# PlanNoa/video_super_resolution

Measured on AMD Instinct MI355X. Metric: HR frames/sec, 1080p->4K x4 VSR (LR 540x960 -> 2160x3840), VSR.forward end-to-end, higher is better.
Workload: dtype f16

## Files before the change

__graft_entry__.py:

```python
import os

os.environ.setdefault("MIOPEN_FIND_MODE", "2")
os.environ.setdefault("MIOPEN_DEBUG_ENABLE_AI_IMMED_MODE_FALLBACK", "0")
os.environ.setdefault("MIOPEN_LOG_LEVEL", "2")
import subprocess
import sys

ROOT = os.path.dirname(os.path.abspath(__file__))
if ROOT not in sys.path:
    sys.path.insert(0, ROOT)


def build() -> None:
    from video_super_resolution_amd import _lib
    _lib.build(verbose=True)
    subprocess.check_call(["make", "-s", "-C", os.path.join(ROOT, "oracle"), "_build/liboracle_native.so"])
    import video_super_resolution_amd
    missing = [s for s in _lib.declared_symbols() if not hasattr(_lib.load(), s)]
    if missing:
        raise RuntimeError(f"libvsr_hip.so lacks {missing}")
    xmissing = [s for s in _lib.declared_symbols() + _lib.declared_symbols(xcheck=True) if not hasattr(_lib.load_xcheck(), s)]
    if xmissing:
        raise RuntimeError(f"libvsr_hip_xcheck.so lacks {xmissing}")
    s3missing = [s for s in _lib.declared_symbols(s3=True) if not hasattr(_lib.load_s3(), s)]
    if s3missing:
        raise RuntimeError(f"libvsr_hip_s3.so lacks {s3missing}")
    s3tmissing = [s for s in _lib.declared_symbols(s3t=True) if not hasattr(_lib.load_s3t(), s)]
    if s3tmissing:
        raise RuntimeError(f"libvsr_hip_s3t.so lacks {s3tmissing}")


def smoke() -> None:
    import numpy as np
    import torch
    from oracle import native, vsr_oracle
    from video_super_resolution_amd import SRProjectionModule, ops
    from video_super_resolution_amd.weights import fill_module_

    assert torch.cuda.is_available(), "smoke() needs cuda:0"
    torch.cuda.set_device(0)
    rs = np.random.RandomState(0)
    img = rs.randn(1, 3, 32, 48).astype(np.float32)
    flow = (rs.randn(1, 2, 32, 48) * 4).astype(np.float32)
    got = ops.resample2d(torch.from_numpy(img).cuda(), torch.from_numpy(flow).cuda()).cpu().numpy()
    assert np.array_equal(got, native.resample2d(img, flow)), "flow warp differs from the oracle"

    sr = fill_module_(SRProjectionModule().eval(), seed=0, prefix="model.")
    x = torch.from_numpy(rs.randint(0, 256, (8, 3, 10, 12)).astype(np.float32))
    with torch.no_grad():
        ref = vsr_oracle.sr_forward({k: v for k, v in sr.state_dict().items()}, x).numpy()
    sr = sr.cuda()
    errs = {}
    for precision, bar in (("fp32", 1e-3), ("fp16", 5e-3)):
        sr.precision = precision
        out = sr(x.cuda()).cpu().numpy()
        errs[precision] = np.abs(out - ref).max() / np.abs(ref).max()
        assert errs[precision] < bar, f"SR forward ({precision}) differs from the oracle: {errs[precision]}"
    print(f"smoke ok: warp bit-exact, SR forward rel err fp32 {errs['fp32']:.2e}, fp16/MFMA {errs['fp16']:.2e}")


if __name__ == "__main__":
    build()
    if len(sys.argv) > 1 and sys.argv[1] == "smoke":
        smoke()
```

video_super_resolution_amd/_lib.py:

```python
from __future__ import annotations

import ctypes
import os
import re
import subprocess

import torch

_PKG = os.path.dirname(os.path.abspath(__file__))
_ROOT = os.path.dirname(_PKG)
LIB_PATH = os.path.join(_PKG, "libvsr_hip.so")
XLIB_PATH = os.path.join(_PKG, "libvsr_hip_xcheck.so")
HEADER_PATH = os.path.join(_ROOT, "include", "vsr_hip.h")
XHEADER_PATH = os.path.join(_ROOT, "include", "vsr_hip_xcheck.h")
GLIB_PATH = os.path.join(_PKG, "libvsr_hip_grad.so")
GHEADER_PATH = os.path.join(_ROOT, "include", "vsr_hip_grad.h")
S3LIB_PATH = os.path.join(_PKG, "libvsr_hip_s3.so")
S3HEADER_PATH = os.path.join(_ROOT, "include", "vsr_hip_s3.h")
S3TLIB_PATH = os.path.join(_PKG, "libvsr_hip_s3t.so")
S3THEADER_PATH = os.path.join(_ROOT, "include", "vsr_hip_s3t.h")
_lib = None
_xlib = None
_glib = None
_s3lib = None
_s3tlib = None
_use_x = os.environ.get("VSR_USE_XCHECK", "0") == "1" or bool(os.environ.get("VSR_TUNING", "").strip())


class VsrHipError(RuntimeError):
    pass


def build(verbose: bool = False) -> str:
    cmd = ["make", "-j4", "-C", os.path.join(_PKG, "csrc")]
    if not verbose:
        cmd.insert(1, "-s")
    subprocess.check_call(cmd)
    return LIB_PATH


def declared_symbols(xcheck: bool = False, grad: bool = False, s3: bool = False, s3t: bool = False) -> list:
    with open(S3THEADER_PATH if s3t else S3HEADER_PATH if s3 else GHEADER_PATH if grad else XHEADER_PATH if xcheck else HEADER_PATH) as f:
        text = re.sub(r"/\*.*?\*/", "", f.read(), flags=re.S)
    return sorted(set(re.findall(r"\b(vsr_[a-z0-9_]+)\s*\(", text)))


def _dlopen(path: str) -> ctypes.CDLL:
    if not os.path.exists(path):
        raise VsrHipError(
            f"{path} is missing: build it with `python -c 'import __graft_entry__ as g; g.build()'` "
            "(there is no CPU fallback for the device path)")
    return ctypes.CDLL(path)


def _open(path: str) -> ctypes.CDLL:
    lib = _dlopen(path)
    lib.vsr_last_error.restype = ctypes.c_char_p
    lib.vsr_last_route.restype = ctypes.c_char_p
    for fn in ("vsr_sr_query", "vsr_train_corr_dw_ws_floats", "vsr_train_prelu_bwd_ws_floats"):
        getattr(lib, fn).restype = ctypes.c_size_t
    if lib.vsr_abi_version() != 3:
        raise VsrHipError(f"{os.path.basename(path)}: ABI version mismatch")
    return lib


def load_xcheck() -> ctypes.CDLL:
    global _xlib
    if _xlib is None:
        lib = _open(XLIB_PATH)
        for t in os.environ.get("VSR_TUNING", "").split(","):
            if t.strip():
                lib.vsr_conv2d_tuning(int(t))
        _xlib = lib
    return _xlib


def load_grad() -> ctypes.CDLL:
    global _glib
    if _glib is None:
        lib = _dlopen(GLIB_PATH)
        lib.vsr_grad_last_error.restype = ctypes.c_char_p
        lib.vsr_last_error = lib.vsr_grad_last_error
        if lib.vsr_grad_abi_version() != 1:
            raise VsrHipError(f"{os.path.basename(GLIB_PATH)}: ABI version mismatch")
        _glib = lib
    return _glib


def load_s3() -> ctypes.CDLL:
    global _s3lib
    if _s3lib is None:
        lib = _dlopen(S3LIB_PATH)
        lib.vsr_s3_last_error.restype = ctypes.c_char_p
        lib.vsr_last_error = lib.vsr_s3_last_error
        lib.vsr_s3_query.restype = ctypes.c_size_t
        if lib.vsr_s3_abi_version() != 1:
            raise VsrHipError(f"{os.path.basename(S3LIB_PATH)}: ABI version mismatch")
        _s3lib = lib
    return _s3lib


def load_s3t() -> ctypes.CDLL:
    global _s3tlib
    if _s3tlib is None:
        lib = _dlopen(S3TLIB_PATH)
        lib.vsr_s3t_last_error.restype = ctypes.c_char_p
        lib.vsr_last_error = lib.vsr_s3t_last_error
        lib.vsr_s3t_query.restype = ctypes.c_size_t
        if lib.vsr_s3t_abi_version() != 1:
            raise VsrHipError(f"{os.path.basename(S3TLIB_PATH)}: ABI version mismatch")
        _s3tlib = lib
    return _s3tlib


def load() -> ctypes.CDLL:
    global _lib
    if _use_x:
        return load_xcheck()
    if _lib is None:
        _lib = _open(LIB_PATH)
    return _lib


class xcheck:

    def __enter__(self):
        global _use_x
        self._old, _use_x = _use_x, True
        return load_xcheck()

    def __exit__(self, *exc):
        global _use_x
        _use_x = self._old
        return False


Q_UTD_BLOB_BYTES, Q_UTD_STRIP_WIDTH, Q_UTD_S2_BLOB_BYTES, Q_UTD_S2_STRIP_WIDTH, Q_TAIL_S2_BLOB_BYTES = range(5)
Q_S3_BLOB_BYTES, Q_S3_STRIP_WIDTH = range(2)
Q_S3T_BLOB_BYTES, Q_S3T_BLOB_FOLD_BYTES, Q_S3T_STRIP_WIDTH = range(3)


def check(rc: int, what: str = "", lib=None) -> None:
    if rc != 0:
        libs = [lib] if lib is not None else [l for l in (load(), _lib, _xlib) if l is not None]
        msgs = []
        for l in libs:
            m = l.vsr_last_error().decode("utf-8", "replace")
            if m and m not in msgs:
                msgs.append(m)
        raise VsrHipError(f"{what or 'vsr'} failed ({rc}): {' | '.join(msgs)}")


def dptr(t: torch.Tensor, dtype=torch.float32) -> ctypes.c_void_p:
    if not t.is_cuda:
        raise VsrHipError("device path called with a CPU tensor (no CPU fallback exists)")
    if t.dtype != dtype:
        raise VsrHipError(f"expected {dtype}, got {t.dtype}")
    if not t.is_contiguous():
        raise VsrHipError("tensor must be contiguous")
    return ctypes.c_void_p(t.data_ptr())


def optr(t, dtype=torch.float32):
    return ctypes.c_void_p(0) if t is None else dptr(t, dtype)


_raw_stream = getattr(torch._C, "_cuda_getCurrentRawStream", None)


def raw_stream(index=None) -> int:
    if _raw_stream is not None:
        return _raw_stream(torch._C._cuda_getDevice() if index is None else index)
    return torch.cuda.current_stream(index).cuda_stream


def stream() -> ctypes.c_void_p:
    return ctypes.c_void_p(raw_stream())


def _first_cuda_tensor(objs):
    for o in objs:
        if isinstance(o, torch.Tensor):
            if o.is_cuda:
                return o
        elif isinstance(o, (list, tuple)):
            t = _first_cuda_tensor(o)
            if t is not None:
                return t
    return None


def on_device(fn):
    import functools

    @functools.wraps(fn)
    def wrapped(*args, **kwargs):
        t = _first_cuda_tensor(args)
        if t is None:
            t = _first_cuda_tensor(tuple(kwargs.values()))
        if t is None or t.device.index == torch.cuda.current_device():
            return fn(*args, **kwargs)
        with torch.cuda.device(t.device):
            return fn(*args, **kwargs)
    return wrapped


def cf(v: float) -> ctypes.c_float:
    return ctypes.c_float(float(v))


class _ChainStage(ctypes.Structure):
    _fields_ = [("inp", ctypes.c_void_p * 2), ("w", ctypes.c_void_p * 2), ("ldw", ctypes.c_int * 2), ("w_prev", ctypes.c_void_p),
                ("ldw_prev", ctypes.c_int), ("bias", ctypes.c_void_p), ("cmap", ctypes.c_void_p), ("slope", ctypes.c_float),
                ("out", ctypes.c_void_p)]


class Chain1x1(ctypes.Structure):
    _fields_ = [("nstages", ctypes.c_int), ("stage", _ChainStage * 3)]


_ROUTE_BATCH = os.environ.get("VSR_ROUTE_BATCH", "1") != "0"


class route_batch:

    def __init__(self, num: int, den: int):
        self.num, self.den = int(num), int(den)
        self.on = self.den > 0 and self.num > 0 and self.num != self.den and _ROUTE_BATCH

    def __enter__(self):
        if self.on:
            check(load().vsr_conv2d_route_batch(self.num, self.den), "conv2d_route_batch")
        return self

    def __exit__(self, *exc):
        if self.on:
            load().vsr_conv2d_route_batch(0, 0)
        return False


class serial_streams:
    on = False

    def __init__(self, enable: bool = True):
        self.enable = bool(enable)

    def __enter__(self):
        self._old, serial_streams.on = serial_streams.on, serial_streams.on or self.enable
        return self

    def __exit__(self, *exc):
        serial_streams.on = self._old
        return False


class EventTimer:

    def __init__(self):
        self.enabled = False
        self.only = None
        self._pairs = {}

    def reset(self):
        self._pairs = {}

    def start(self, name: str):
        if not self.enabled or (self.only is not None and name not in self.only):
            return None
        a = torch.cuda.Event(enable_timing=True)
        b = torch.cuda.Event(enable_timing=True)
        a.record()
        self._pairs.setdefault(name, []).append((a, b))
        return b

    @staticmethod
    def stop(tok):
        if tok is not None:
            tok.record()

    def summary(self):
        return {k: (len(v), sum(a.elapsed_time(b) for a, b in v) / len(v)) for k, v in self._pairs.items()}


TIMER = EventTimer()


class RouteLog:

    def __init__(self):
        self.enabled = False
        self.calls = []

    def note(self, label: str):
        if self.enabled:
            self.calls.append((label, load().vsr_last_route().decode()))

    def note_as(self, label: str, route: str):
        if self.enabled:
            self.calls.append((label, route))

    def last(self) -> str:
        return load().vsr_last_route().decode()

    def histogram(self):
        h = {}
        for _, r in self.calls:
            h[r] = h.get(r, 0) + 1
        return h


ROUTES = RouteLog()
```

video_super_resolution_amd/trunk_exec.py:

```python
from __future__ import annotations

import ctypes
import os

import torch
import torch.nn as nn
import torch.nn.functional as F

from . import _lib as L
from . import ops
from .depth import HOURGLASS
from .igemm import (ACT_LEAKY, ACT_NONE, ACT_RELU, HConv, HConvPairS2, HConvStem, HDeconv4s2, HFlowHead, HHourglassFront, SegMap, cached_zeros,
                    pad32, pool2x2, resize_add, to_nhwc_half)


def _fold(conv: nn.Conv2d, bn):
    w = conv.weight.detach().float()
    b = conv.bias.detach().float() if conv.bias is not None else torch.zeros(w.shape[0], device=w.device)
    if bn is not None:
        scale = torch.rsqrt(bn.running_var.float() + bn.eps)
        if bn.affine:
            scale = scale * bn.weight.detach().float()
        shift = -bn.running_mean.float() * scale
        if bn.affine:
            shift = shift + bn.bias.detach().float()
        w = w * scale.view(-1, 1, 1, 1)
        b = b * scale + shift
    return w, b


def _nchw(x):
    return x.permute(0, 3, 1, 2)


def _nhwc(x):
    return x.permute(0, 2, 3, 1).contiguous()


class _Inception:

    def __init__(self, mod):
        b0 = mod[0]
        w0, bb0 = _fold(b0[0], b0[1])
        ws, bs, self.kconvs = [], [], []
        mids, outs = [], []
        for j in (1, 2, 3):
            br = mod[j]
            w1, b1 = _fold(br[0], br[1])
            ws.append(w1)
            bs.append(b1)
            mids.append(w1.shape[0])
            wk, bk = _fold(br[3], br[4])
            outs.append(wk.shape[0])
            self.kconvs.append((wk, bk, br[3].kernel_size[0]))
        self.M = sum(mids)
        self.o0 = w0.shape[0]
        self.ctot = self.o0 + sum(outs)
        self.width = pad32(self.M + self.ctot)
        self.first = HConv(torch.cat(ws + [w0], 0), torch.cat(bs + [bb0], 0), act=ACT_RELU)
        packed = []
        moff, ooff = 0, self.M + self.o0
        for (wk, bk, k), mid, o in zip(self.kconvs, mids, outs):
            packed.append((HConv(wk, bk, pad=(k - 1) // 2, act=ACT_RELU), moff, ooff))
            moff += mid
            ooff += o
        self.kconvs = packed
        self.cin = w0.shape[1]

    dense_thin = os.environ.get("VSR_DENSE_THIN", "1") != "0"

    def branches(self, buf):
        if self.dense_thin and all(conv.cout == 16 for conv, _, _ in self.kconvs) and self.o0 == 16:
            N, H, W, _ = buf.shape
            outs = torch.empty((len(self.kconvs), N, H, W, 16), dtype=torch.float16, device=buf.device)
            for j, (conv, moff, _) in enumerate(self.kconvs):
                conv(buf, out=outs[j], out_coff=0, in_coff=moff)
            return SegMap([(buf, self.M)] + [(outs[j], 0) for j in range(len(self.kconvs))]), 0, self.ctot
        for conv, moff, ooff in self.kconvs:
            conv(buf, out=buf, out_coff=ooff, in_coff=moff)
        return buf, self.M, self.ctot

    def __call__(self, x, in_coff):
        N, H, W, _ = x.shape
        buf = torch.empty((N, H, W, self.width), dtype=torch.float16, device=x.device)
        if self.width != self.M + self.ctot:
            buf[..., self.M + self.ctot:] = 0
        self.first(x, out=buf, out_coff=0, in_coff=in_coff)
        return self.branches(buf)


class HourglassExec:
    fused_front = os.environ.get("VSR_HG_FRONT", "1") != "0"

    def __init__(self, netg: nn.Sequential):
        self.prog = self._build(HOURGLASS, netg)
        self.front = self._match_front(self.prog)

    @staticmethod
    def _match_front(prog):
        try:
            items = prog[1]
            stem, lvl = items[0], items[1]
            fan = lvl[1][0]
            arm_a, arm_b = fan[1]
            ok = (stem[0] == "stem" and stem[2] == 128 and lvl[0] == "S" and lvl[1][1] == "+" and len(lvl[1]) == 2 and fan[0] == "M" and
                  arm_a[0] == "S" and arm_a[1][0] == "max" and arm_b[0] == "S" and len(arm_b[1]) == 1 and arm_b[1][0][0] == "I" and
                  arm_b[1][0][1].cin == 128)
            return HHourglassFront(stem[1], arm_b[1][0][1].first) if ok else None
        except (IndexError, TypeError, ValueError, AttributeError):
            return None

    def _build(self, node, mod):
        if isinstance(node, str):
            return node
        tag = node[0]
        if tag == "S":
            items, children = [], list(mod)
            i = 0
            while i < len(node[1]):
                ch = node[1][i]
                if isinstance(ch, tuple) and ch[0] == "conv":
                    bn = children[i + 1] if i + 1 < len(children) and isinstance(children[i + 1], nn.BatchNorm2d) else None
                    j = i + (2 if bn is not None else 1)
                    relu = j < len(children) and isinstance(children[j], nn.ReLU)
                    w, b = _fold(children[i], bn)
                    if w.shape[1] <= 4 and w.shape[3] <= 8:
                        items.append(("stem", HConvStem(w, b, pad=ch[4], act=ACT_RELU if relu else ACT_NONE), ch[2]))
                    else:
                        items.append(("conv", HConv(w, b, pad=ch[4], act=ACT_RELU if relu else ACT_NONE), ch[2]))
                    i = j + (1 if relu else 0)
                    continue
                items.append(self._build(ch, children[i]))
                i += 1
            return ("S", items)
        if tag == "M":
            return ("M", [self._build(c, m) for c, m in zip(node[1], mod)])
        if tag == "I":
            return ("I", _Inception(mod))
        raise ValueError(node)

    def _side(self, dev, level):
        if L.serial_streams.on:
            return torch.cuda.current_stream(dev)
        key = (dev.type, dev.index)
        if getattr(self, "_side_key", None) != key:
            self._side_streams, self._side_key = {}, key
        if level not in self._side_streams:
            self._side_streams[level] = torch.cuda.Stream(device=dev)
        return self._side_streams[level]

    def _fan_out(self, subs, x, coff, c, level):
        if len(subs) != 2 or not self.concurrent:
            return [self._run(sub, x, coff, c, level + 1) for sub in subs]
        cur = torch.cuda.current_stream(x.device)
        side = self._side(x.device, level)
        side.wait_stream(cur)
        with torch.cuda.stream(side):
            first = self._run(subs[0], x, coff, c, level + 1)
            first[0].record_stream(cur)
        x.record_stream(side)
        second = self._run(subs[1], x, coff, c, level + 1)
        cur.wait_stream(side)
        return [first, second]

    concurrent = os.environ.get("VSR_HOURGLASS_STREAMS", "0") == "1"
    defer_up = True

    def _run(self, node, x, coff, c, level=0):
        if node == "max" or node == "avg":
            return pool2x2(x, coff, c, 0 if node == "max" else 1), 0, c
        if node == "up":
            return resize_add(x, coff, c, (2 * x.shape[1], 2 * x.shape[2])), 0, c
        tag = node[0]
        if tag == "conv":
            if node[2] == 1:
                N, H, W, _ = x.shape
                Ho, Wo = node[1].out_hw(H, W)
                out = node[1](x, in_coff=coff, out=torch.empty((N, Ho, Wo, 1), dtype=torch.float16, device=x.device))
            else:
                out = node[1](x, in_coff=coff)
            return out, 0, node[2]
        if tag == "stem":
            return node[1](x), 0, node[2]
        if tag == "I":
            buf, m, ctot = node[1](x, coff)
            return buf, m, ctot
        if tag == "S":
            items = node[1]
            for i, ch in enumerate(items):
                if ch == "+":
                    a, ca, na = x[0][:3]
                    b, cb, nb = x[1][:3]
                    a_up, b_up = len(x[0]) > 3, len(x[1]) > 3
                    out_hw = (b.shape[1] << b_up, b.shape[2] << b_up)
                    x, coff, c = resize_add(a, ca, nb, out_hw, b, cb, up2=a_up, b_up2=b_up), 0, nb
                elif isinstance(ch, tuple) and ch[0] == "M":
                    x = self._fan_out(ch[1], x, coff, c, level)
                elif ch == "up" and i == len(items) - 1 and self.defer_up:
                    return x, coff, c, "up2"
                else:
                    x, coff, c = self._run(ch, x, coff, c, level)
            return x, coff, c
        raise ValueError(node)

    @L.on_device
    @torch.no_grad()
    def __call__(self, frames_nhwc3: torch.Tensor) -> torch.Tensor:
        k, h, w, _ = frames_nhwc3.shape
        stem_first = self.prog[0] == "S" and isinstance(self.prog[1][0], tuple) and self.prog[1][0][0] == "stem"
        x = cached_zeros(self, "in", (k, h, w, 4 if stem_first else 32), frames_nhwc3.device)
        x[..., :3] = frames_nhwc3
        if self.front is not None and self.fused_front and h >= 2 and w >= 2:
            out, coff, c = self._run_fused_front(x)
        else:
            out, coff, c = self._run(self.prog, x, 0, 32)
        return out[..., coff:coff + 1].permute(0, 3, 1, 2).float()

    def _run_fused_front(self, x4):
        k, h, w, _ = x4.shape
        items = self.prog[1]
        arm_a, arm_b = items[1][1][0][1]
        inc = arm_b[1][0][1]
        buf = torch.empty((k, h, w, inc.width), dtype=torch.float16, device=x4.device)
        if inc.width != inc.M + inc.ctot:
            buf[..., inc.M + inc.ctot:] = 0
        pooled = torch.empty((k, h // 2, w // 2, 128), dtype=torch.float16, device=x4.device)
        self.front(x4, buf, pooled)
        a = self._run(("S", arm_a[1][1:]), pooled, 0, 128, 1)
        x, coff, c = self._run(("S", ["+"]), [a, inc.branches(buf)], 0, 0)
        return self._run(("S", items[2:]), x, coff, c)


def _cv(seq, stride=1, act=ACT_LEAKY, cin_pad=None):
    conv = seq[0] if isinstance(seq, nn.Sequential) else seq
    k = conv.kernel_size[0]
    return HConv(conv.weight, conv.bias, stride=conv.stride[0], pad=(k - 1) // 2, act=act, slope=0.1, cin_pad=cin_pad)


class _Refine:
    fused_heads = os.environ.get("VSR_FLOW_HEADS", "1") != "0"

    def __init__(self, net, with_inter: bool):
        self.with_inter = with_inter
        self.pred6 = _cv(net.predict_flow6, act=ACT_NONE)
        self.levels = []
        prev_pred = net.predict_flow6
        for lvl, cin_cat in ((5, 1026), (4, 770), (3, 386), (2, 194)):
            dec = getattr(net, f"deconv{lvl}")[0]
            up = getattr(net, f"upsampled_flow{lvl + 1}_to_{lvl}")
            item = dict(deconv=HDeconv4s2(dec.weight, dec.bias, act=ACT_LEAKY),
                        upflow=HDeconv4s2(up.weight, up.bias, act=ACT_NONE),
                        cat=pad32(cin_cat), dec_c=dec.weight.shape[1])
            pred = getattr(net, f"predict_flow{lvl}")
            if with_inter:
                item["inter"] = _cv(getattr(net, f"inter_conv{lvl}"), act=ACT_NONE, cin_pad=pad32(cin_cat))
                item["pred"] = _cv(pred, act=ACT_NONE)
            else:
                item["pred"] = _cv(pred, act=ACT_NONE, cin_pad=pad32(cin_cat))
            item["head_in"] = HFlowHead(prev_pred.weight, prev_pred.bias, up.weight, up.bias,
                                        cin_pad=None if (with_inter or lvl == 5) else self.levels[-1]["cat"])
            prev_pred = pred
            self.levels.append(item)
        self.head_last = HFlowHead(prev_pred.weight, prev_pred.bias, cin_pad=None if with_inter else self.levels[-1]["cat"])

    def alloc_cat(self, idx, N, H, W, dev):
        return cached_zeros(self, f"cat{idx}", (N, H, W, self.levels[idx]["cat"]), dev)

    def __call__(self, c6, cats, enc_c):
        if not self.fused_heads:
            flow = self.pred6(c6)
            src = c6
            for i, lv in enumerate(self.levels):
                cat = cats[i]
                lv["deconv"](src, out=cat, out_coff=enc_c[i])
                lv["upflow"](flow, out=cat, out_coff=enc_c[i] + lv["dec_c"])
                flow = lv["pred"](lv["inter"](cat)) if self.with_inter else lv["pred"](cat)
                src = cat
            return flow
        src = head_src = c6
        for i, lv in enumerate(self.levels):
            cat = cats[i]
            lv["deconv"](src, out=cat, out_coff=enc_c[i])
            lv["head_in"](head_src, up_out=cat, up_coff=enc_c[i] + lv["dec_c"])
            src = cat
            head_src = lv["inter"](cat) if self.with_inter else cat
        return self.head_last(head_src)


class _FlowNetSExec:
    def __init__(self, net, cin):
        c1 = net.conv1[0] if isinstance(net.conv1, nn.Sequential) else net.conv1
        self.conv1 = HConvPairS2(c1.weight, c1.bias, pad=(c1.kernel_size[0] - 1) // 2, act=ACT_LEAKY, slope=0.1) \
            if cin <= 16 and c1.stride[0] == 2 else _cv(net.conv1, cin_pad=pad32(cin))
        self.pair_input = isinstance(self.conv1, HConvPairS2)
        self.names = ["conv2", "conv3", "conv3_1", "conv4", "conv4_1", "conv5", "conv5_1", "conv6", "conv6_1"]
        self.convs = {n: _cv(getattr(net, n)) for n in self.names}
        self.refine = _Refine(net, with_inter=False)

    def __call__(self, x):
        N, H, W, _ = x.shape
        dev = x.device
        c1 = self.conv1(x)
        h2, w2 = H // 4, W // 4
        cats = [self.refine.alloc_cat(i, N, H >> (5 - i), W >> (5 - i), dev) for i in range(4)]
        self.convs["conv2"](c1, out=cats[3], out_coff=0)
        self.convs["conv3_1"](self.convs["conv3"](cats[3]), out=cats[2], out_coff=0)
        self.convs["conv4_1"](self.convs["conv4"](cats[2]), out=cats[1], out_coff=0)
        self.convs["conv5_1"](self.convs["conv5"](cats[1]), out=cats[0], out_coff=0)
        c6 = self.convs["conv6_1"](self.convs["conv6"](cats[0]))
        return self.refine(c6, cats, [512, 512, 256, 128])


class _FlowNetCExec:
    def __init__(self, net):
        c1 = net.conv1[0] if isinstance(net.conv1, nn.Sequential) else net.conv1
        self.conv1 = HConvStem(c1.weight, c1.bias, stride=c1.stride[0], pad=(c1.kernel_size[0] - 1) // 2, act=ACT_LEAKY, slope=0.1)
        self.conv2, self.conv3 = _cv(net.conv2), _cv(net.conv3)
        self.redir = _cv(net.conv_redir)
        self.conv3_1 = _cv(net.conv3_1, cin_pad=pad32(473))
        self.names = ["conv4", "conv4_1", "conv5", "conv5_1", "conv6", "conv6_1"]
        self.convs = {n: _cv(getattr(net, n)) for n in self.names}
        self.refine = _Refine(net, with_inter=False)

    def __call__(self, x6, both=None):
        B, H, W, _ = x6.shape
        dev = x6.device
        if both is None:
            both = cached_zeros(self, "both", (2 * B, H, W, 4), dev)
            both[:B, ..., :3] = x6[..., 0:3]
            both[B:, ..., :3] = x6[..., 3:6]
        c2 = self.conv2(self.conv1(both))
        c3 = self.conv3(c2)
        a3, b3 = c3[:B], c3[B:]
        h8, w8 = H // 8, W // 8
        cat31 = cached_zeros(self, "cat31", (B, h8, w8, pad32(473)), dev)
        self.redir(a3, out=cat31, out_coff=0)
        L.check(L.load().vsr_flownetc_corr_nhwc_f16(L.dptr(a3, torch.float16), L.dptr(b3, torch.float16), L.dptr(cat31, torch.float16),
                                                    cat31.shape[3], 32, B, h8, w8, c3.shape[3], L.stream()), "flownetc_corr")
        cats = [self.refine.alloc_cat(i, B, H >> (5 - i), W >> (5 - i), dev) for i in range(4)]
        cats[3][..., :128] = c2[:B]
        self.conv3_1(cat31, out=cats[2], out_coff=0)
        self.convs["conv4_1"](self.convs["conv4"](cats[2]), out=cats[1], out_coff=0)
        self.convs["conv5_1"](self.convs["conv5"](cats[1]), out=cats[0], out_coff=0)
        c6 = self.convs["conv6_1"](self.convs["conv6"](cats[0]))
        return self.refine(c6, cats, [512, 512, 256, 128])


class _FlowNetSDExec:
    def __init__(self, net):
        self.conv0 = _cv(net.conv0, cin_pad=32)
        self.names = ["conv1", "conv1_1", "conv2", "conv2_1", "conv3", "conv3_1", "conv4", "conv4_1", "conv5", "conv5_1",
                      "conv6", "conv6_1"]
        self.convs = {n: _cv(getattr(net, n)) for n in self.names}
        self.refine = _Refine(net, with_inter=True)

    def __call__(self, x6):
        N, H, W, _ = x6.shape
        dev = x6.device
        c = self.convs
        c0 = self.conv0(x6)
        c1 = c["conv1_1"](c["conv1"](c0))
        cats = [self.refine.alloc_cat(i, N, H >> (5 - i), W >> (5 - i), dev) for i in range(4)]
        c["conv2_1"](c["conv2"](c1), out=cats[3], out_coff=0)
        c["conv3_1"](c["conv3"](cats[3]), out=cats[2], out_coff=0)
        c["conv4_1"](c["conv4"](cats[2]), out=cats[1], out_coff=0)
        c["conv5_1"](c["conv5"](cats[1]), out=cats[0], out_coff=0)
        c6 = c["conv6_1"](c["conv6"](cats[0]))
        return self.refine(c6, cats, [512, 512, 256, 128])


class _FusionExec:
    def __init__(self, net):
        self.conv0 = _cv(net.conv0, cin_pad=32)
        self.conv1, self.conv1_1 = _cv(net.conv1), _cv(net.conv1_1)
        self.conv2, self.conv2_1 = _cv(net.conv2), _cv(net.conv2_1)
        self.pred2 = _cv(net.predict_flow2, act=ACT_NONE)
        self.deconv1 = HDeconv4s2(net.deconv1[0].weight, net.deconv1[0].bias, act=ACT_LEAKY)
        self.up21 = HDeconv4s2(net.upsampled_flow2_to_1.weight, net.upsampled_flow2_to_1.bias)
        self.inter1 = _cv(net.inter_conv1, act=ACT_NONE, cin_pad=pad32(162))
        self.pred1 = _cv(net.predict_flow1, act=ACT_NONE)
        self.deconv0 = HDeconv4s2(net.deconv0[0].weight, net.deconv0[0].bias, act=ACT_LEAKY, cin_pad=pad32(162))
        self.up10 = HDeconv4s2(net.upsampled_flow1_to_0.weight, net.upsampled_flow1_to_0.bias)
        self.inter0 = _cv(net.inter_conv0, act=ACT_NONE, cin_pad=pad32(82))
        self.pred0 = _cv(net.predict_flow0, act=ACT_NONE)
        self.head2 = HFlowHead(net.predict_flow2.weight, net.predict_flow2.bias, net.upsampled_flow2_to_1.weight, net.upsampled_flow2_to_1.bias)

    def __call__(self, x11):
        N, H, W, _ = x11.shape
        dev = x11.device
        cat0 = cached_zeros(self, "cat0", (N, H, W, pad32(82)), dev)
        cat1 = cached_zeros(self, "cat1", (N, H // 2, W // 2, pad32(162)), dev)
        self.conv0(x11, out=cat0, out_coff=0)
        self.conv1_1(self.conv1(cat0), out=cat1, out_coff=0)
        c2 = self.conv2_1(self.conv2(cat1))
        if _Refine.fused_heads:
            self.head2(c2, up_out=cat1, up_coff=160)
            self.deconv1(c2, out=cat1, out_coff=128)
        else:
            flow2 = self.pred2(c2)
            self.deconv1(c2, out=cat1, out_coff=128)
            self.up21(flow2, out=cat1, out_coff=160)
        flow1 = self.pred1(self.inter1(cat1))
        self.deconv0(cat1, out=cat0, out_coff=64)
        self.up10(flow1, out=cat0, out_coff=80)
        return self.pred0(self.inter0(cat0))


class FlowNet2Exec:
    def __init__(self, net):
        self.div_flow = net.div_flow
        self.c = _FlowNetCExec(net.flownetc)
        self.s1 = _FlowNetSExec(net.flownets_1, 12)
        self.s2 = _FlowNetSExec(net.flownets_2, 12)
        self.sd = _FlowNetSDExec(net.flownets_d)
        self.fusion = _FusionExec(net.flownetfusion)

    def _sd_stream(self, dev):
        if L.serial_streams.on:
            return torch.cuda.current_stream(dev)
        key = (dev.type, dev.index)
        if getattr(self, "_sd_key", None) != key:
            self._sd_side, self._sd_key = torch.cuda.Stream(device=dev), key
        return self._sd_side

    @staticmethod
    def _flow_nchw(t):
        return t[..., :2].permute(0, 3, 1, 2).float()

    @L.on_device
    @torch.no_grad()
    def __call__(self, inputs):
        B, _, _, H, W = inputs.shape
        frames = inputs.float().permute(0, 2, 3, 4, 1).reshape(2 * B, H, W, 3).contiguous()
        out = []
        for b0 in range(0, B, 4):
            nb = min(4, B - b0)
            out.append(self.run_pairs(frames[2 * b0:2 * (b0 + nb)], [(2 * i, 2 * i + 1) for i in range(nb)]))
        return self._flow_nchw(out[0] if len(out) == 1 else torch.cat(out, 0))

    @L.on_device
    @torch.no_grad()
    def run_pairs(self, frames, pairs, crop=None):
        lib = L.load()
        B = len(pairs)
        F_, h, w, _ = frames.shape
        y0, x0, H, W = crop or (0, 0, h, w)
        dev = frames.device
        frames = frames.contiguous()
        x = torch.empty((B, 6, H, W), dtype=torch.float32, device=dev)
        x6 = torch.empty((B, H, W, 32), dtype=torch.float16, device=dev)
        both = torch.empty((2 * B, H, W, 4), dtype=torch.float16, device=dev)
        ws = torch.empty(B * 128 * 3, dtype=torch.float32, device=dev)
        ia = (ctypes.c_int * B)(*[p[0] for p in pairs])
        ib = (ctypes.c_int * B)(*[p[1] for p in pairs])
        L.check(lib.vsr_flownet_prepare_pairs(L.dptr(frames), F_, h, w, ia, ib, B, y0, x0, H, W, L.dptr(ws), L.dptr(x),
                                              L.dptr(x6, torch.float16), L.dptr(both, torch.float16), L.stream()), "flownet_prepare_pairs")
        if not (self.s1.pair_input and self.s2.pair_input):
            raise NotImplementedError("FlowNetS stems other than 12 -> 64, stride 2 (the reference's)")

        def warp_cat(flow2):
            cat = torch.empty((B, H, W, 16), dtype=torch.float16, device=dev)
            L.check(lib.vsr_flownet_up_warp_concat16_f16(L.dptr(x), L.dptr(flow2, torch.float16), flow2.shape[3], 1, L.cf(self.div_flow),
                                                         L.cf(1.0 / self.div_flow), L.dptr(cat, torch.float16), B, H, W, L.stream()),
                    "up_warp_concat16")
            return cat
        main = torch.cuda.current_stream(dev)
        side = self._sd_stream(dev) if os.environ.get("VSR_FLOWSD_STREAM", "1") != "0" else main
        side.wait_stream(main)
        with torch.cuda.stream(side):
            sd2 = self.sd(x6)
            sd2.record_stream(main)
        x6.record_stream(side)
        s1_in = warp_cat(self.c(x6, both))
        s2_in = warp_cat(self.s1(s1_in))
        s22 = self.s2(s2_in)
        main.wait_stream(side)
        x11 = torch.empty((B, H, W, 32), dtype=torch.float16, device=dev)
        L.check(lib.vsr_flownet_fusion_input_f16(L.dptr(x), L.dptr(sd2, torch.float16), sd2.shape[3], L.dptr(s22, torch.float16), s22.shape[3],
                                                 L.cf(self.div_flow), L.dptr(x11, torch.float16), B, H, W, L.stream()), "fusion_input")
        return self.fusion(x11)


class OSVOSExec:
    def __init__(self, net):
        self.stages = []
        for si, stage in enumerate(net.stages):
            items = []
            for m in stage:
                if isinstance(m, nn.MaxPool2d):
                    items.append("M")
                elif isinstance(m, nn.Conv2d):
                    items.append(HConvStem(m.weight, m.bias, pad=1, act=ACT_RELU) if m.in_channels == 3 else
                                 HConv(m.weight, m.bias, pad=1, act=ACT_RELU))
            self.stages.append(items)
        self.side = [HConv(m.weight, m.bias, pad=1, act=ACT_NONE) for m in net.side_prep]
        fw = net.fuse.weight.detach().float().view(-1)
        self.up_s = [m.stride[0] for m in net.upscale]
        self.weff = [torch.einsum("iokl,o->kli", m.weight.detach().float(), fw[16 * b:16 * b + 16]).contiguous().half()
                     for b, m in enumerate(net.upscale)]
        self.fuse_b = float(net.fuse.bias.detach())

    @L.on_device
    @torch.no_grad()
    def __call__(self, x_nchw):
        N = x_nchw.shape[0]
        hh, ww = x_nchw.shape[-2:]
        x = to_nhwc_half(x_nchw, 4)
        sides = []
        for si, items in enumerate(self.stages):
            for it in items:
                x = pool2x2(x, 0, x.shape[3], 2) if it == "M" else it(x)
            if si > 0:
                hs, ws = x.shape[1], x.shape[2]
                sides.append(self.side[si - 1](x, out=torch.empty((N, hs, ws, 16), dtype=torch.float16, device=x.device)))
        nb = len(sides)
        out = torch.empty((N, 1, hh, ww), dtype=torch.float32, device=x.device)
        vp = ctypes.c_void_p * nb
        ip = ctypes.c_int * nb
        L.check(L.load().vsr_osvos_fuse_f16(vp(*[t.data_ptr() for t in sides]), ip(*[t.shape[1] for t in sides]),
                                            ip(*[t.shape[2] for t in sides]), sides[0].shape[3], vp(*[t.data_ptr() for t in self.weff]),
                                            ip(*self.up_s), nb, L.cf(self.fuse_b), L.dptr(out), N, hh, ww, L.stream()), "osvos_fuse")
        return out


class VGGFeatExec:

    def __init__(self, seq):
        self.items = []
        for m in seq:
            if isinstance(m, nn.MaxPool2d):
                self.items.append("M")
            elif isinstance(m, nn.Conv2d):
                self.items.append(HConvStem(m.weight, m.bias, pad=1, act=ACT_RELU) if m.in_channels == 3 else
                                  HConv(m.weight, m.bias, pad=1, act=ACT_RELU))

    @L.on_device
    @torch.no_grad()
    def __call__(self, x_nchw):
        x = to_nhwc_half(x_nchw.float().contiguous(), 4)
        for it in self.items:
            x = pool2x2(x, 0, x.shape[3], 0) if it == "M" else it(x)
        return x.permute(0, 3, 1, 2).float()


class TrunkExecCache:

    def __init__(self, master: nn.Module, factory):
        self.master, self.factory = master, factory
        self._exec, self._key, self._mods = None, None, None

    def key(self):
        if self._mods is None:
            self._mods = [m for m in self.master.modules() if m._parameters or m._buffers]
        return tuple((t.data_ptr(), t._version) for m in self._mods for d in (m._parameters, m._buffers) for t in d.values() if t is not None)

    def get(self):
        key = self.key()
        if self._exec is None or key != self._key:
            self._exec, self._key = self.factory(self.master), key
        return self._exec
```

Before: 43.80.

## Fuse inception 3/5/7 branch convolutions into one persistent pipelined kernel

Adds a new HIP kernel that runs an inception module's three same-shape branch convolutions (k=7, 5, 3) in one persistent launch. Each stage prefetches the next branch's (or next tile's) input patch while it computes the current one on MFMA. The Python executor probes once per shape that the per-branch convs would route to patch kernels, caches that result, and then switches to the fused launch. The aim is to cut launch count and keep the loads overlapped across branches. The cost is a new library, fixed LDS and grid sizing at two blocks per CU, and a first call that always takes the unfused path.

```diff
diff --git a/__graft_entry__.py b/__graft_entry__.py
--- a/__graft_entry__.py
+++ b/__graft_entry__.py
@@ -28,6 +28,9 @@
     s3tmissing = [s for s in _lib.declared_symbols(s3t=True) if not hasattr(_lib.load_s3t(), s)]
     if s3tmissing:
         raise RuntimeError(f"libvsr_hip_s3t.so lacks {s3tmissing}")
+    incmissing = [s for s in _lib.declared_symbols(inc=True) if not hasattr(_lib.load_inc(), s)]
+    if incmissing:
+        raise RuntimeError(f"libvsr_hip_inc.so lacks {incmissing}")
 
 
 def smoke() -> None:
diff --git a/include/vsr_hip_inc.h b/include/vsr_hip_inc.h
--- /dev/null
+++ b/include/vsr_hip_inc.h
@@ -0,0 +1,25 @@
+#ifndef VSR_HIP_INC_H
+#define VSR_HIP_INC_H
+
+#include <stddef.h>
+
+#include "vsr_hip.h"
+
+#ifdef __cplusplus
+extern "C" {
+#endif
+
+#define VSR_INC_ABI_VERSION 1
+
+int vsr_inc_abi_version(void);
+const char* vsr_inc_last_error(void);
+
+int vsr_inc_branches_f16(const void* in, int in_ld, const int* k, const int* in_coff, const void* const* w_packed, const float* const* bias,
+                         void* const* out, const int* out_ld, const int* out_coff, int N, int H, int W, int cin, int cout, int cout_pad,
+                         int act, float slope, vsr_stream_t stream);
+
+#ifdef __cplusplus
+}
+#endif
+
+#endif
diff --git a/video_super_resolution_amd/_lib.py b/video_super_resolution_amd/_lib.py
--- a/video_super_resolution_amd/_lib.py
+++ b/video_super_resolution_amd/_lib.py
@@ -4,6 +4,7 @@
 import os
 import re
 import subprocess
+import threading
 
 import torch
 
@@ -23,7 +24,10 @@
 _xlib = None
 _glib = None
 _s3lib = None
+INCLIB_PATH = os.path.join(_PKG, "libvsr_hip_inc.so")
+INCHEADER_PATH = os.path.join(_ROOT, "include", "vsr_hip_inc.h")
 _s3tlib = None
+_inclib = None
 _use_x = os.environ.get("VSR_USE_XCHECK", "0") == "1" or bool(os.environ.get("VSR_TUNING", "").strip())
 
 
@@ -39,8 +43,8 @@
     return LIB_PATH
 
 
-def declared_symbols(xcheck: bool = False, grad: bool = False, s3: bool = False, s3t: bool = False) -> list:
-    with open(S3THEADER_PATH if s3t else S3HEADER_PATH if s3 else GHEADER_PATH if grad else XHEADER_PATH if xcheck else HEADER_PATH) as f:
+def declared_symbols(xcheck: bool = False, grad: bool = False, s3: bool = False, s3t: bool = False, inc: bool = False) -> list:
+    with open(INCHEADER_PATH if inc else S3THEADER_PATH if s3t else S3HEADER_PATH if s3 else GHEADER_PATH if grad else XHEADER_PATH if xcheck else HEADER_PATH) as f:
         text = re.sub(r"/\*.*?\*/", "", f.read(), flags=re.S)
     return sorted(set(re.findall(r"\b(vsr_[a-z0-9_]+)\s*\(", text)))
 
@@ -113,6 +117,18 @@
     return _s3tlib
 
 
+def load_inc() -> ctypes.CDLL:
+    global _inclib
+    if _inclib is None:
+        lib = _dlopen(INCLIB_PATH)
+        lib.vsr_inc_last_error.restype = ctypes.c_char_p
+        lib.vsr_last_error = lib.vsr_inc_last_error
+        if lib.vsr_inc_abi_version() != 1:
+            raise VsrHipError(f"{os.path.basename(INCLIB_PATH)}: ABI version mismatch")
+        _inclib = lib
+    return _inclib
+
+
 def load() -> ctypes.CDLL:
     global _lib
     if _use_x:
@@ -228,14 +244,22 @@
         self.num, self.den = int(num), int(den)
         self.on = self.den > 0 and self.num > 0 and self.num != self.den and _ROUTE_BATCH
 
+    _state = threading.local()
+
+    @staticmethod
+    def current():
+        return getattr(route_batch._state, "v", (0, 0))
+
     def __enter__(self):
         if self.on:
             check(load().vsr_conv2d_route_batch(self.num, self.den), "conv2d_route_batch")
+            route_batch._state.v = (self.num, self.den)
         return self
 
     def __exit__(self, *exc):
         if self.on:
             load().vsr_conv2d_route_batch(0, 0)
+            route_batch._state.v = (0, 0)
         return False
 
 
diff --git a/video_super_resolution_amd/csrc/conv_inception.hip b/video_super_resolution_amd/csrc/conv_inception.hip
--- /dev/null
+++ b/video_super_resolution_amd/csrc/conv_inception.hip
@@ -0,0 +1,260 @@
+#include <cstdint>
+
+#include "conv_patch.h"
+
+#include "../../include/vsr_hip_inc.h"
+
+namespace {
+
+using vsrc::ConvP;
+using vsrc::f4;
+using vsrc::h8;
+using vsrc::P8_H;
+using vsrc::P8_R;
+using vsrc::P8_W;
+
+typedef unsigned int u4v __attribute__((ext_vector_type(4)));
+
+constexpr int MT = 2;
+constexpr int npc(int kh) { return ((P8_H + kh - 1) * (P8_W + kh - 1) * 4 + 255) / 256; }
+constexpr int NPC_MAX = npc(7);
+constexpr int LDS_BYTES = (P8_H + 6) * (P8_W + 6) * 64;
+static_assert(LDS_BYTES >= 4 * P8_R * 16 * 32 * MT, "the output tile leaves through the patch memory");
+
+struct IncP {
+    ConvP b[3];
+};
+
+struct Item {
+    int n, oy0, ox0, co0;
+};
+
+struct State {
+    u4v pf[NPC_MAX];
+    f4 acc[P8_R][MT];
+};
+
+__device__ __forceinline__ __amdgpu_buffer_rsrc_t in_rsrc(const ConvP& p, const Item& it) {
+    const int iy0 = it.oy0 - p.pad_y, by = iy0 > 0 ? iy0 : 0;
+    const size_t rem_bytes = (size_t)(p.H - by) * p.W * p.in_ld * 2;
+    return __builtin_amdgcn_make_buffer_rsrc(const_cast<_Float16*>(p.in) + ((size_t)it.n * p.H + by) * p.W * p.in_ld, 0,
+                                             (int)(rem_bytes < 0x7FFFFFF0ull ? rem_bytes : 0x7FFFFFF0ull), 0x00020000);
+}
+
+template <int KH>
+__device__ __forceinline__ int piece_dst(int tid, int k) {
+    constexpr int PH = P8_H + KH - 1, PW = P8_W + KH - 1;
+    const int c4 = tid & 3, pix = (tid >> 2) + 64 * k, px = pix % PW;
+    return pix < PH * PW ? pix * 64 + ((c4 ^ ((px >> 1) & 3)) << 4) : -1;
+}
+template <int KH>
+__device__ __forceinline__ unsigned piece_off(const ConvP& p, const Item& it, int tid, int k) {
+    constexpr int PH = P8_H + KH - 1, PW = P8_W + KH - 1;
+    const int c4 = tid & 3, pix = (tid >> 2) + 64 * k, py = pix / PW, px = pix - py * PW;
+    const int iy0 = it.oy0 - p.pad_y, by = iy0 > 0 ? iy0 : 0;
+    const int iy = iy0 + py, ix = it.ox0 - p.pad_x + px;
+    const bool ok = pix < PH * PW && (unsigned)iy < (unsigned)p.H && (unsigned)ix < (unsigned)p.W;
+    const unsigned ld2 = (unsigned)p.in_ld * 2, row2 = (unsigned)p.W * ld2;
+    return ok ? (unsigned)(iy - by) * row2 + (unsigned)ix * ld2 + (unsigned)p.in_coff * 2 + c4 * 16 : 0xFFFFFFFFu;
+}
+
+template <int KH>
+__device__ __forceinline__ void issue(State& s, const ConvP& p, const Item& it, __amdgpu_buffer_rsrc_t rs, int ch, bool valid, int tid, int k0, int k1) {
+    const unsigned coff = (unsigned)ch * 64u;
+#pragma unroll
+    for (int k = k0; k < k1; ++k)
+        if (k < npc(KH)) {
+            const unsigned off = piece_off<KH>(p, it, tid, k);
+            s.pf[k] = __builtin_amdgcn_raw_buffer_load_b128(rs, off == 0xFFFFFFFFu || !valid ? 0xFFFFFFFFu : off + coff, 0, 0);
+        }
+}
+
+template <int KH, int KHN>
+__device__ __forceinline__ void stage(State& s, unsigned char* psm, const ConvP& p, const Item& it, int ch, bool first, bool last, const ConvP& pn,
+                                      const Item& itn, int chn, bool valid, int tid, int lane, int wv) {
+    constexpr int PW = P8_W + KH - 1, NP = npc(KH), NPN = npc(KHN);
+    constexpr bool AHEAD = KH <= 5;
+    asm volatile("" : "+v"(tid));
+    lane = tid & 63;
+    const int l15 = lane & 15, g = lane >> 4;
+    const int nchunk = p.cin >> 5;
+    const int ry0 = P8_R * (wv >> 1), cx0 = 16 * (wv & 1);
+    const _Float16* const wbase_p = p.wpk + ((size_t)ch * p.cout_pad + it.co0 + l15) * 32 + 8 * g;
+    const size_t wtap = (size_t)nchunk * p.cout_pad * 32;
+    auto wfrag = [&](int ky, int kx, int mt) __attribute__((always_inline)) {
+        return *reinterpret_cast<const h8*>(wbase_p + (size_t)(ky * KH + kx) * wtap + 16 * 32 * mt);
+    };
+    h8 A[KH][MT];
+#pragma unroll
+    for (int ky = 0; ky < KH; ++ky)
+#pragma unroll
+        for (int mt = 0; mt < MT; ++mt) A[ky][mt] = wfrag(ky, 0, mt);
+    __syncthreads();
+#pragma unroll
+    for (int k = 0; k < NP; ++k) {
+        const int dst = piece_dst<KH>(tid, k);
+        if (dst >= 0) *reinterpret_cast<u4v*>(psm + dst) = s.pf[k];
+    }
+    __syncthreads();
+    const __amdgpu_buffer_rsrc_t rsn = in_rsrc(pn, itn);
+    if (first) {
+#pragma unroll
+        for (int r = 0; r < P8_R; ++r)
+#pragma unroll
+            for (int mt = 0; mt < MT; ++mt) s.acc[r][mt] = f4{0.0f, 0.0f, 0.0f, 0.0f};
+    }
+#pragma unroll
+    for (int kx = 0; kx < KH; ++kx) {
+        h8 An[AHEAD ? KH : 1][MT];
+        if (AHEAD && kx + 1 < KH) {
+#pragma unroll
+            for (int ky = 0; ky < KH; ++ky)
+#pragma unroll
+                for (int mt = 0; mt < MT; ++mt) An[ky][mt] = wfrag(ky, kx + 1, mt);
+        }
+        issue<KHN>(s, pn, itn, rsn, chn, valid, tid, kx * NPN / KH, (kx + 1) * NPN / KH);
+        const int px = cx0 + l15 + kx;
+        const unsigned char* src = psm + (ry0 * PW + px) * 64 + ((g ^ ((px >> 1) & 3)) << 4);
+#pragma unroll
+        for (int pr = 0; pr < KH + P8_R - 1; ++pr) {
+            const h8 bf = *reinterpret_cast<const h8*>(src + pr * PW * 64);
+#pragma unroll
+            for (int r = 0; r < P8_R; ++r) {
+                const int ky = pr - r;
+                if (ky < 0 || ky >= KH) continue;
+#pragma unroll
+                for (int mt = 0; mt < MT; ++mt) s.acc[r][mt] = __builtin_amdgcn_mfma_f32_16x16x32_f16(A[ky][mt], bf, s.acc[r][mt], 0, 0, 0);
+            }
+            const int kd = pr - (P8_R - 1);
+            if (!AHEAD && kx + 1 < KH && kd >= 0 && kd < KH) {
+#pragma unroll
+                for (int mt = 0; mt < MT; ++mt) A[kd][mt] = wfrag(kd, kx + 1, mt);
+            }
+        }
+        if (AHEAD && kx + 1 < KH) {
+#pragma unroll
+            for (int ky = 0; ky < KH; ++ky)
+#pragma unroll
+                for (int mt = 0; mt < MT; ++mt) A[ky][mt] = An[ky][mt];
+        }
+        asm volatile("" ::: "memory");
+        __builtin_amdgcn_sched_barrier(0);
+    }
+    if (!last) return;
+    __syncthreads();
+    const long long wbase = (((long long)it.n * p.outH + (it.oy0 + ry0) * p.oy_mul + p.oy_off) * p.outW + (it.ox0 + cx0) * p.ox_mul + p.ox_off) * p.out_ld;
+    const int rstride = p.oy_mul * p.outW * p.out_ld, cstride = p.ox_mul * p.out_ld;
+    const int rows_ok = p.Ho - (it.oy0 + ry0), cols_ok = p.Wo - (it.ox0 + cx0);
+    vsrc::patch_epilogue<MT, P8_R>(p, psm + wv * (P8_R * 16 * 32 * MT), it.co0, lane, [&](int r, int mt) { return s.acc[r][mt]; },
+                                   [&](int r, int li) { return r < rows_ok && li < cols_ok ? wbase + r * rstride + li * cstride : -1ll; });
+}
+
+template <int NCH>
+__global__ void __launch_bounds__(256, 2) k_conv_inception(const IncP P, int tiles_x, int tiles_y, int ncb, int nwork) {
+    extern __shared__ __attribute__((aligned(16))) unsigned char psm[];
+    const int tid = threadIdx.x, lane = tid & 63, wv = __builtin_amdgcn_readfirstlane(tid >> 6);
+    auto decode = [&](int w) {
+        Item it;
+        const int cb = w % ncb, t = w / ncb;
+        const int tx = t % tiles_x, t2 = t / tiles_x, ty = t2 % tiles_y;
+        it.n = t2 / tiles_y;
+        it.oy0 = ty * P8_H; it.ox0 = tx * P8_W; it.co0 = cb * 16 * MT;
+        return it;
+    };
+    int w = blockIdx.x;
+    if (w >= nwork) return;
+    State s;
+    Item cur = decode(w);
+    issue<7>(s, P.b[0], cur, in_rsrc(P.b[0], cur), 0, true, tid, 0, npc(7));
+    while (true) {
+        const int w2 = w + (int)gridDim.x;
+        const bool have_next = w2 < nwork;
+        const Item nxt = have_next ? decode(w2) : cur;
+        if (NCH == 2) {
+            stage<7, 7>(s, psm, P.b[0], cur, 0, true, false, P.b[0], cur, 1, true, tid, lane, wv);
+            stage<7, 5>(s, psm, P.b[0], cur, 1, false, true, P.b[1], cur, 0, true, tid, lane, wv);
+            stage<5, 5>(s, psm, P.b[1], cur, 0, true, false, P.b[1], cur, 1, true, tid, lane, wv);
+            stage<5, 3>(s, psm, P.b[1], cur, 1, false, true, P.b[2], cur, 0, true, tid, lane, wv);
+            stage<3, 3>(s, psm, P.b[2], cur, 0, true, false, P.b[2], cur, 1, true, tid, lane, wv);
+            stage<3, 7>(s, psm, P.b[2], cur, 1, false, true, P.b[0], nxt, 0, have_next, tid, lane, wv);
+        } else {
+            stage<7, 5>(s, psm, P.b[0], cur, 0, true, true, P.b[1], cur, 0, true, tid, lane, wv);
+            stage<5, 3>(s, psm, P.b[1], cur, 0, true, true, P.b[2], cur, 0, true, tid, lane, wv);
+            stage<3, 7>(s, psm, P.b[2], cur, 0, true, true, P.b[0], nxt, 0, have_next, tid, lane, wv);
+        }
+        if (!have_next) break;
+        cur = nxt;
+        w = w2;
+    }
+}
+
+bool ranges_overlap(const void* a, size_t na, const void* b, size_t nb) {
+    const uintptr_t a0 = reinterpret_cast<uintptr_t>(a), b0 = reinterpret_cast<uintptr_t>(b);
+    return a0 < b0 + nb && b0 < a0 + na;
+}
+
+bool slices_clash(const void* a, int lda, int c0, int n0, const void* b, int ldb, int c1, int n1, size_t pix) {
+    if (a == b && lda == ldb) return c0 < c1 + n1 && c1 < c0 + n0;
+    return ranges_overlap(a, pix * lda * 2, b, pix * ldb * 2);
+}
+
+}
+
+extern "C" {
+
+int vsr_inc_abi_version(void) { return VSR_INC_ABI_VERSION; }
+const char* vsr_inc_last_error(void) { return vsr::err_buf(); }
+
+int vsr_inc_branches_f16(const void* in, int in_ld, const int* k, const int* in_coff, const void* const* w_packed, const float* const* bias,
+                         void* const* out, const int* out_ld, const int* out_coff, int N, int H, int W, int cin, int cout, int cout_pad,
+                         int act, float slope, vsr_stream_t stream) {
+    VSR_REQUIRE(in && k && in_coff && w_packed && bias && out && out_ld && out_coff, "inc_branches: null pointer");
+    for (int j = 0; j < 3; ++j) VSR_REQUIRE(w_packed[j] && out[j], "inc_branches: null pointer (branch %d)", j);
+    VSR_REQUIRE(N > 0 && N <= 65535 && H >= 12 && W >= 16, "inc_branches: bad shape (N %d, H %d, W %d)", N, H, W);
+    VSR_REQUIRE(act >= 0 && act <= 2, "inc_branches: activation %d", act);
+    int order[3] = {-1, -1, -1};
+    for (int j = 0; j < 3; ++j)
+        if (k[j] == 7 || k[j] == 5 || k[j] == 3) order[(7 - k[j]) / 2] = j;
+    if (order[0] < 0 || order[1] < 0 || order[2] < 0)
+        return vsr::fail(VSR_E_UNSUPPORTED, "inc_branches: unsupported k-set (%d, %d, %d): the build walks 3, 5 and 7", k[0], k[1], k[2]);
+    if ((cin != 32 && cin != 64) || (cout_pad != 32 && cout_pad != 64) || cout <= 0 || cout > cout_pad)
+        return vsr::fail(VSR_E_UNSUPPORTED, "inc_branches: %d -> %d (padded %d) channels: builds exist for 32 / 64 -> 32 / 64", cin, cout, cout_pad);
+    VSR_REQUIRE((in_ld & 7) == 0 && (reinterpret_cast<uintptr_t>(in) & 15) == 0, "inc_branches: input rows of %d channels are not 16-byte aligned", in_ld);
+    const size_t pix = (size_t)N * H * W;
+    VSR_REQUIRE(pix < (1ull << 31), "inc_branches: %zu output pixels exceed the kernel's 32-bit pixel index", pix);
+    if ((unsigned long long)(7 + 16) * W * in_ld * 2 >= (1ull << 31))
+        return vsr::fail(VSR_E_UNSUPPORTED, "inc_branches: a patch of %d-channel rows of %d pixels exceeds the 2 GiB the staging addresses", in_ld, W);
+    for (int j = 0; j < 3; ++j) {
+        VSR_REQUIRE((in_coff[j] & 7) == 0 && in_coff[j] >= 0 && in_coff[j] + cin <= in_ld, "inc_branches: input slice [%d,+%d) of %d channels", in_coff[j], cin, in_ld);
+        VSR_REQUIRE(out_coff[j] >= 0 && out_ld[j] > 0 && out_coff[j] + cout <= out_ld[j], "inc_branches: output slice [%d,+%d) of %d channels", out_coff[j], cout,
+                    out_ld[j]);
+        for (int i = 0; i < 3; ++i)
+            VSR_REQUIRE(!slices_clash(out[j], out_ld[j], out_coff[j], cout, in, in_ld, in_coff[i], cin, pix),
+                        "inc_branches: output slice of branch %d overlaps the input slice of branch %d", j, i);
+        for (int i = 0; i < j; ++i)
+            VSR_REQUIRE(!slices_clash(out[j], out_ld[j], out_coff[j], cout, out[i], out_ld[i], out_coff[i], cout, pix),
+                        "inc_branches: output slices of branches %d and %d overlap", i, j);
+    }
+    IncP P;
+    for (int o = 0; o < 3; ++o) {
+        const int j = order[o];
+        ConvP& p = P.b[o];
+        p = ConvP{};
+        p.in = (const _Float16*)in; p.wpk = (const _Float16*)w_packed[j]; p.bias = bias[j]; p.out = (_Float16*)out[j];
+        p.in_ld = in_ld; p.in_coff = in_coff[j]; p.out_ld = out_ld[j]; p.out_coff = out_coff[j];
+        p.N = N; p.H = H; p.W = W; p.cin = cin; p.Ho = H; p.Wo = W; p.cout = cout; p.cout_pad = cout_pad;
+        p.kh = p.kw = k[j]; p.stride = p.stride_x = 1; p.pad_y = p.pad_x = (k[j] - 1) / 2;
+        p.outH = H; p.outW = W; p.oy_mul = p.ox_mul = 1; p.oy_off = p.ox_off = 0;
+        p.act = act; p.slope = slope; p.ws = nullptr; p.splits = 1; p.nphase = 0;
+    }
+    const int tiles_x = (int)vsr::cdiv(W, P8_W), tiles_y = (int)vsr::cdiv(H, P8_H), ncb = cout_pad / (16 * MT);
+    const long long nwork = (long long)N * tiles_x * tiles_y * ncb;
+    if (nwork >= (1ll << 30)) return vsr::fail(VSR_E_ARG, "inc_branches: %lld work items", nwork);
+    auto kern = cin == 64 ? &k_conv_inception<2> : &k_conv_inception<1>;
+    const long long resident = 256LL * 2;
+    const unsigned grid = (unsigned)(nwork < resident ? nwork : resident);
+    hipLaunchKernelGGL(kern, dim3(grid), dim3(256), LDS_BYTES, vsr::S(stream), P, tiles_x, tiles_y, ncb, (int)nwork);
+    return vsr::launched("inc_branches_f16");
+}
+
+}
diff --git a/video_super_resolution_amd/trunk_exec.py b/video_super_resolution_amd/trunk_exec.py
--- a/video_super_resolution_amd/trunk_exec.py
+++ b/video_super_resolution_amd/trunk_exec.py
@@ -76,9 +76,57 @@
             for j, (conv, moff, _) in enumerate(self.kconvs):
                 conv(buf, out=outs[j], out_coff=0, in_coff=moff)
             return SegMap([(buf, self.M)] + [(outs[j], 0) for j in range(len(self.kconvs))]), 0, self.ctot
+        if self.fused_branches and self._fusable and not L._use_x:
+            ok = self._patch_routed(buf)
+            if ok is None:
+                return buf, self.M, self.ctot
+            if ok:
+                self._launch_fused(buf)
+                return buf, self.M, self.ctot
         for conv, moff, ooff in self.kconvs:
             conv(buf, out=buf, out_coff=ooff, in_coff=moff)
         return buf, self.M, self.ctot
+
+    fused_branches = os.environ.get("VSR_INCEPTION_FUSED", "1") != "0"
+    _PATCH_ROUTES = ("patch_r8<", "patch_lw<", "patch_pf<")
+    _routes = {}
+
+    @property
+    def _fusable(self):
+        convs = [c for c, _, _ in self.kconvs]
+        return (sorted(c.kh for c in convs) == [3, 5, 7] and all(c.kh == c.kw and c.stride == 1 for c in convs)
+                and len({(c.cin_pad, c.cout, c.cout_pad, c.act) for c in convs}) == 1
+                and convs[0].cin_pad in (32, 64) and convs[0].cout_pad in (32, 64))
+
+    def _patch_routed(self, buf):
+        N, H, W, _ = buf.shape
+        c0 = self.kconvs[0][0]
+        key = (N, L.route_batch.current(), H, W, c0.cin_pad, c0.cout_pad)
+        ok = _Inception._routes.get(key)
+        if ok is not None:
+            return ok
+        ok = True
+        for conv, moff, ooff in self.kconvs:
+            conv(buf, out=buf, out_coff=ooff, in_coff=moff)
+            ok = ok and L.ROUTES.last().startswith(self._PATCH_ROUTES)
+        _Inception._routes[key] = ok
+        return None
+
+    def _launch_fused(self, buf):
+        N, H, W, ld = buf.shape
+        convs = [c for c, _, _ in self.kconvs]
+        c0 = convs[0]
+        ia, va = ctypes.c_int * 3, ctypes.c_void_p * 3
+        name = f"inception N{N} {H}x{W} c{c0.cin_pad}->{c0.cout} k{'+'.join(str(c.kh) for c in convs)}"
+        tok = L.TIMER.start(name) if L.TIMER.enabled else None
+        bp = L.dptr(buf, torch.float16)
+        lib = L.load_inc()
+        L.check(lib.vsr_inc_branches_f16(
+            bp, ld, ia(*[c.kh for c in convs]), ia(*[m for _, m, _ in self.kconvs]), va(*[L.dptr(c.w, torch.float16).value for c in convs]),
+            va(*[L.optr(c.b).value for c in convs]), va(bp.value, bp.value, bp.value), ia(ld, ld, ld), ia(*[o for _, _, o in self.kconvs]),
+            N, H, W, c0.cin_pad, c0.cout, c0.cout_pad, c0.act, L.cf(c0.slope), L.stream()), "inc_branches_f16", lib=lib)
+        L.TIMER.stop(tok)
+        L.ROUTES.note_as(name, f"inception<{c0.cin_pad // 32}>")
 
     def __call__(self, x, in_coff):
         N, H, W, _ = x.shape
```

After: 44.03, median of 6. No clear change (+0.5%).
